# eyedealism/flexible-LLM-sharding

Measured on AMD Instinct MI355X. Metric: tokens/sec + peak GPU mem, Llama-2-70B layer_num_per_shard=1 at 1/2/4/8 MI355X, higher is better.
Workload: dtype fp16

## Files before the change

csrc/include/fls.h:

```cpp
#pragma once
#include <stdint.h>
#include <stddef.h>

#ifdef __cplusplus
extern "C" {
#endif

typedef void* fls_stream_t;

int   fls_rt_version(void);
void* fls_pinned_alloc(uint64_t bytes);
int   fls_pinned_free(void* p);
void* fls_host_device_ptr(void* p);
int   fls_pinned_register(void* p, uint64_t bytes);
int   fls_pinned_unregister(void* p);
int   fls_memcpy_async(void* dst, const void* src, uint64_t bytes, int kind, fls_stream_t s);
int64_t fls_pread_into(const char* path, uint64_t offset, uint64_t bytes, void* dst, int nthreads);
int64_t fls_pwrite_from(const char* path, uint64_t offset, uint64_t bytes, const void* src,
                        int nthreads, int truncate);
int   fls_gather_blocks(void* dst, const void* src, uint64_t block_bytes, const int64_t* src_block,
                        int64_t n_blocks, int nthreads);
void* fls_st_open(const char* path);
int   fls_st_count(void* h);
int   fls_st_info(void* h, int i, char* name, int name_cap, char* dtype, int dtype_cap,
// ... 50 lines not shown
int fls_moe_router_route(const void* h, int ldh, const void* wr, int ldw, int T, int H, int E, int k, int norm,
                         int round16, int* ids, float* w, fls_stream_t s);
int fls_moe_plan_scratch(int n, int E);
int fls_moe_plan(const int* ids, int n, int k, int E, int* offs, int* tiles, int* rows, int* dest, int* bhist,
                 fls_stream_t s);
int fls_moe_gemm(const void* A, const void* W, void* C, int M_bound, int N, int K, int lda, int ldw, int ldc, int epi,
                 const int* tiles, const int* offs, const int* rows, int n_groups, long long wstride, int a_rows,
                 fls_stream_t s);
int fls_moe_combine(const void* y, int ldy, const int* ids, const int* dest, const float* w, void* x, int ldx, int T,
                    int k, int H, const void* sh, int ldsh, fls_stream_t s);
int fls_gemm_set_order(int order);
int fls_gemm_set_mid_bn(int bn);
int fls_gemm_set_mid_waves(int waves);
int fls_gemm_set_mid_rows(int rows);
int fls_gemm_set_mid(int on);
int fls_attention_set_hpb(int hpb);
int fls_attention_set_split(int ns);
int fls_attention_set_persistent(int on);
int fls_attention(const void* qkv, void* out, const int* work, int n_items, int n_q_heads,
                  int n_kv_heads, int head_dim, int ld_qkv, int ld_out, float scale, const void* kv0,
                  int ld_kv0, const int* seg_lo, int q_block, const int* work2, const int* r2win,
                  void* ws, unsigned long long ws_bytes, int n_rows, fls_stream_t s);
int fls_attention_window(const void* qkv, void* out, const int* work, int n_items, int n_q_heads,
                         int n_kv_heads, int head_dim, int ld_qkv, int ld_out, float scale, const void* kv0,
                         int ld_kv0, const int* seg_lo, int q_block, const int* work2, const int* r2win,
                         void* ws, unsigned long long ws_bytes, int n_rows, const int* r0_lo,
                         const int* r0_item, fls_stream_t s);
int fls_headnorm_rope(void* x, int ldx, int rows, int n_q, int n_k, const void* qn, const void* kn, const int* pos,
                      const float* cos_t, const float* sin_t, int hd, float eps, fls_stream_t s);
int fls_rmsnorm(const void* x, const void* w, void* y, const int* row_idx, int rows, int H,
// ... 30 lines not shown
```

csrc/kernels/common.h:

```cpp
#pragma once
#include <hip/hip_runtime.h>
#include <stdint.h>

typedef _Float16 half_t;
typedef _Float16 half8 __attribute__((ext_vector_type(8)));
typedef _Float16 half4 __attribute__((ext_vector_type(4)));
typedef float floatx4 __attribute__((ext_vector_type(4)));
typedef short s16x4 __attribute__((vector_size(8)));

#define LDS_AS __attribute__((address_space(3)))
#define GLB_AS __attribute__((address_space(1)))

constexpr int WAVE = 64;

__device__ __forceinline__ floatx4 mfma16x16x32(half8 a, half8 b, floatx4 c) {
  return __builtin_amdgcn_mfma_f32_16x16x32_f16(a, b, c, 0, 0, 0);
}

__device__ __forceinline__ void mfma_acc_inplace_ordered(floatx4& c, const half8& a, const half8& b) {
  asm volatile("v_mfma_f32_16x16x32_f16 %0, %1, %2, %0" : "+a"(c) : "v"(a), "v"(b) : "memory");
}

__device__ __forceinline__ void glds16(const void* gsrc, void* lds_wave_base) {
  __builtin_amdgcn_global_load_lds((const GLB_AS void*)gsrc, (LDS_AS void*)lds_wave_base, 16, 0, 0);
// ... 6 lines not shown

__device__ __forceinline__ float warp_max(float v) {
#pragma unroll
  for (int o = 32; o > 0; o >>= 1) v = fmaxf(v, __shfl_xor(v, o, 64));
  return v;
}

__device__ __forceinline__ float warp_sum(float v) {
#pragma unroll
  for (int o = 32; o > 0; o >>= 1) v += __shfl_xor(v, o, 64);
  return v;
}

__device__ __forceinline__ float fast_exp2(float x) { return __builtin_amdgcn_exp2f(x); }

__device__ __forceinline__ float silu(float x) { return x / (1.0f + __expf(-x)); }

#define FLS_CHECK_LAUNCH()                                  \
  do {                                                      \
    hipError_t _e = hipGetLastError();                      \
    if (_e != hipSuccess) return (int)_e;                   \
  } while (0)
```

csrc/kernels/gemm.hip:

```cpp
#include "gemm_v10.h"

namespace {

template <int EPI>
__global__ __launch_bounds__(256) void gemm_nt_generic(const half_t* __restrict__ A, const half_t* __restrict__ W,
                                                     half_t* __restrict__ C, int M, int N, int K, int lda, int ldw,
                                                     int ldc, Epi ep) {
  const int lane = threadIdx.x & 63, wave = threadIdx.x >> 6;
  const int fr = lane & 15, grp = lane >> 4;
  const int m0 = blockIdx.x * 32;
  const bool rope128 = EPI == FLS_EPI_ROPE;
  const int gbase = blockIdx.y * 256 + (wave >> 1) * 128;
  int ncol[4];
#pragma unroll
  for (int t = 0; t < 4; ++t) ncol[t] = gbase + sub_col(rope128, wave & 1, t);
  floatx4 acc[2][4];
#pragma unroll
  for (int u = 0; u < 2; ++u)
#pragma unroll
    for (int t = 0; t < 4; ++t) acc[u][t] = floatx4{0.f, 0.f, 0.f, 0.f};
  for (int k0 = 0; k0 < K; k0 += 32) {
    half8 wf[4], xf[2];
    const int kb = k0 + grp * 8;
#pragma unroll
// ... 269 lines not shown
      const half4 b = *(const half4*)(ep.bias + col);
#pragma unroll
      for (int r = 0; r < 4; ++r) a[r] += (float)b[r];
    }
  };
  auto store4 = [&](const floatx4& a, int col) {
    half4 o;
#pragma unroll
    for (int r = 0; r < 4; ++r) o[r] = (half_t)a[r];
    *(half4*)(C + (size_t)m * ldc + col) = o;
  };
  if constexpr (EPI == FLS_EPI_SWIGLU) {
    const int I = N / 2;
    if (c >= I) return;
    const floatx4 g = sum4(c), u = sum4(I + c);
    floatx4 o;
#pragma unroll
    for (int r = 0; r < 4; ++r) o[r] = silu(g[r]) * u[r];
    store4(o, c);
  } else if constexpr (is_rope(EPI)) {
    const int hd = ep.head_dim, half_hd = hd >> 1, d = c % hd;
    if (c < ep.rope_cols && d >= half_hd) return;
    floatx4 a = sum4(c);
    bias4(a, c);
    if (c >= ep.rope_cols) {
      store4(a, c);
      return;
    }
    floatx4 b = sum4(c + half_hd);
    bias4(b, c + half_hd);
    const int p = ep.pos[m];
    const floatx4 cs = *(const floatx4*)(ep.cos_t + (size_t)p * half_hd + d);
    const floatx4 sn = *(const floatx4*)(ep.sin_t + (size_t)p * half_hd + d);
// ... 194 lines not shown
    return 0;
  }
  const int tiles = (int)tiles256;
  const int tiles_m = (M + BM - 1) / BM, tiles_n = N / BN;
  int order = g_order;
  if (order == 0) order = auto_order(tiles_m, tiles_n);
  Epi e = ep;
  e.order = order;
  launch_main<EPI>(tiles, A, W, C, M, N, K, lda, ldw, ldc, e, s);
  FLS_CHECK_LAUNCH();
  return 0;
}

}

extern "C" int fls_kernels_version(void) { return 41; }

extern "C" int fls_gemm_set_order(int order) {
  const int old = g_order;
  g_order = order;
  return old;
}

extern "C" int fls_gemm_set_skinny(int mode, int blocks) {
  const int old = g_skinny;
  g_skinny = mode < 0 ? 0 : mode > 2 ? 2 : mode;
  g_skinny_blocks = blocks > 0 ? blocks : 0;
  return old;
}

extern "C" int fls_gemm_set_skinny_bn(int bn) {
// ... 41 lines not shown
  const int old = g_mid_waves;
  g_mid_waves = waves == 4 || waves == 8 ? waves : 0;
  return old;
}

extern "C" int fls_gemm_set_mid_rows(int rows) {
  const int old = g_mid_rows;
  g_mid_rows = rows == 64 || rows == 128 ? rows : 0;
  return old;
}

extern "C" int fls_gemm_set_mid(int on) {
  const int old = g_mid;
  g_mid = on ? 1 : 0;
  return old;
}

extern "C" int fls_gemm_v11_try(const void* A, const void* W, void* C, const void* R, int M, int N, int K, int lda,
                                int ldw, int ldc, int ldr, int epi, const int* pos, const float* cos_t,
                                const float* sin_t, int rope_cols, int head_dim, const void* bias,
                                const float* rscale, float alpha, float* ss, int ss_ld, fls_stream_t s);

extern "C" int fls_gemm(const void* A, const void* W, void* C, const void* R, int M, int N, int K, int lda, int ldw,
                        int ldc, int ldr, int epi, const int* pos, const float* cos_t, const float* sin_t,
                        int rope_cols, int head_dim, const void* bias, const float* rscale, float alpha, float* ss,
                        int ss_ld, void* ws, uint64_t ws_bytes, fls_stream_t s) {
  if (M <= 0 || N <= 0 || K <= 0) return 0;
  const int row_exact = (epi & FLS_GEMM_ROW_EXACT) ? 1 : 0;
  epi &= 0xff;
  if (ss && (epi != FLS_EPI_RESID || N % 128 || ss_ld < N / 128)) return -7;
// ... 1 lines not shown
  if ((epi == FLS_EPI_SWIGLU || epi == FLS_EPI_ROPE) && (N % 32)) return -2;
  if (epi == FLS_EPI_ROPE && ((head_dim != 64 && head_dim != 128) || rope_cols % head_dim || N % head_dim))
    return -3;
  {
    const int rc = fls_gemm_v11_try(A, W, C, R, M, N, K, lda, ldw, ldc, ldr, epi, pos, cos_t, sin_t, rope_cols,
                                    head_dim, bias, rscale, alpha, ss, ss_ld, s);
    if (rc) return rc > 0 ? 0 : rc;
  }
  Epi ep{(const half_t*)R, ldr, pos, cos_t, sin_t, rope_cols, head_dim, (const half_t*)bias, N / 2, 0,
         nullptr, nullptr, nullptr, 0, 0};
  ep.rs = rscale;
  ep.alpha = alpha;
  ep.ss = ss;
  ep.ss_ld = ss_ld;
  ep.row_exact = row_exact;
  auto a = (const half_t*)A;
  auto w = (const half_t*)W;
  auto c = (half_t*)C;
  auto st = (hipStream_t)s;
  switch (epi) {
    case FLS_EPI_NONE: return launch<FLS_EPI_NONE>(a, w, c, M, N, K, lda, ldw, ldc, ep, st, ws, ws_bytes);
    case FLS_EPI_RESID: return launch<FLS_EPI_RESID>(a, w, c, M, N, K, lda, ldw, ldc, ep, st, ws, ws_bytes);
    case FLS_EPI_SWIGLU: return launch<FLS_EPI_SWIGLU>(a, w, c, M, N, K, lda, ldw, ldc, ep, st, ws, ws_bytes);
    case FLS_EPI_ROPE:
      return head_dim == 128 ? launch<FLS_EPI_ROPE>(a, w, c, M, N, K, lda, ldw, ldc, ep, st, ws, ws_bytes)
                             : launch<EPI_ROPE64>(a, w, c, M, N, K, lda, ldw, ldc, ep, st, ws, ws_bytes);
  }
  return -1;
}
```

csrc/kernels/gemm_skinny.h:

```cpp
namespace sk {
constexpr int KT = 64;
constexpr int LDS_MAX = 160 * 1024;
template <int RS, int BN>
struct Geo {
  static constexpr bool LATE = BN == 256;
  static constexpr int NSUB = BN / 64;
  static constexpr int XST = RS * 16 * KT * 2;
  static constexpr int WST = BN * KT * 2;
  static constexpr int STG = XST + WST;
  static constexpr int NX = 4 * STG <= LDS_MAX ? 4 : 3 * STG <= LDS_MAX ? 3 : 2;
  static constexpr int DIST = LATE ? NX - 1 : NX - 2;
  static constexpr int QX = RS / 2;
  static constexpr int QW = BN / 32;
  static constexpr int LDS = NX * STG;
  static_assert(DIST >= 1, "at least one K-tile in flight");
};
}

template <int RS, int EPI, int BN>
__global__ __launch_bounds__(256) void gemm_nt_skinny(const half_t* __restrict__ A, const half_t* __restrict__ W,
                                                      half_t* __restrict__ C, int M, int N, int K, int lda, int ldw,
                                                      int ldc, Epi ep) {
  using namespace sk;
  using G = Geo<RS, BN>;
// ... 89 lines not shown
  asm volatile("s_nop 7\n\ts_nop 7\n\ts_nop 7" ::: "memory");
#undef SK_FENCE_ACC

#pragma unroll
  for (int i = 0; i < RS; ++i) {
    const int m = i * 16 + fr;
    if (m >= M) continue;
    const float rsc = row_scale(ep, m);
    if constexpr (EPI == EPI_F32) {
      float* Cf = (float*)C + (size_t)blockIdx.y * ep.part_stride + (size_t)m * ldc;
#pragma unroll
      for (int j = 0; j < NS; ++j) *(floatx4*)(Cf + cbase + 16 * j + 4 * grp) = acc[i][j];
    } else if constexpr (EPI == FLS_EPI_SWIGLU) {
#pragma unroll
      for (int j = 0; j < NS / 2; ++j) {
        half4 o;
#pragma unroll
        for (int r = 0; r < 4; ++r) o[r] = (half_t)(silu(acc[i][j][r] * rsc) * (acc[i][j + NS / 2][r] * rsc));
        *(half4*)(C + (size_t)m * ldc + cbase + 16 * j + 4 * grp) = o;
      }
    } else {
#pragma unroll
      for (int j = 0; j < NS; ++j) {
        const int n = cbase + 16 * j + 4 * grp;
        floatx4 a = acc[i][j] * rsc;
        if (ep.bias) {
          const half4 b = *(const half4*)(ep.bias + n);
#pragma unroll
          for (int r = 0; r < 4; ++r) a[r] += (float)b[r];
        }
        if constexpr (EPI == FLS_EPI_RESID) {
          const half4 rr = *(const half4*)(ep.R + (size_t)m * ep.ldr + n);
#pragma unroll
// ... 113 lines not shown
```

csrc/kernels/gemm_v10.h:

```cpp
#pragma once
#include "common.h"
#include "fls.h"

#include <cstdlib>
#include <type_traits>

namespace {


constexpr int BM = 256, BN = 256, BK = 64;
constexpr int EPI_ROPE64 = 4;
constexpr int EPI_F32 = 6;
constexpr bool is_rope(int epi) { return epi == FLS_EPI_ROPE || epi == EPI_ROPE64; }
constexpr int BUF = 65536;
constexpr int WIMG = 32768;

struct Epi {
  const half_t* R;
  int ldr;
  const int* pos;
  const float* cos_t;
  const float* sin_t;
  int rope_cols;
  int head_dim;
// ... 1 lines not shown
  int gu_rows;
  int order;
  const int* g_tiles;
  const int* g_offs;
  const int* g_rows;
  long long g_wstride;
  int g_n;
  int ksplit;
  int kslice;
  long long part_stride;
  const float* rs = nullptr;
  float alpha = 1.f;
  float* ss = nullptr;
  int ss_ld = 0;
  int row_exact = 0;
};

__device__ __forceinline__ float row_sum_4groups(float v) {
  const auto a = __builtin_amdgcn_permlane32_swap(__float_as_uint(v), __float_as_uint(v), false, false);
  v = __uint_as_float(a[0]) + __uint_as_float(a[1]);
  const auto b = __builtin_amdgcn_permlane16_swap(__float_as_uint(v), __float_as_uint(v), false, false);
  return __uint_as_float(b[0]) + __uint_as_float(b[1]);
}

__device__ __forceinline__ float ss_accum_pair(float sq, const half4& oa, const half4& ob) {
#pragma unroll
  for (int r = 0; r < 4; ++r) {
    const float a = (float)oa[r], b = (float)ob[r];
    sq = __builtin_fmaf(a, a, sq);
    sq = __builtin_fmaf(b, b, sq);
// ... 2 lines not shown
}

__device__ __forceinline__ float row_scale(const Epi& ep, int m) { return ep.rs ? ep.rs[m] : 1.f; }

__device__ __forceinline__ int gu_phys_row(int l, int I) {
  return ((l >> 4) & 1) * I + (l >> 5) * 16 + (l & 15);
}

template <int EPI>
__device__ __forceinline__ void store_pair_off(half_t* __restrict__ C, int ldc, int m, int n_first, int off,
                                               const floatx4& acc_a, const floatx4& acc_b, const Epi& ep) {
  const int c0 = n_first + off;
  if constexpr (EPI == FLS_EPI_SWIGLU) {
    const int oc = n_first / 2 + off;
    const float s = row_scale(ep, m);
    half4 o;
#pragma unroll
    for (int r = 0; r < 4; ++r) o[r] = (half_t)(silu(acc_a[r] * s) * (acc_b[r] * s));
    *(half4*)(C + (size_t)m * ldc + oc) = o;
    return;
  } else {
    const float s = row_scale(ep, m);
    floatx4 a = acc_a * s, b = acc_b * s;
    if (ep.bias) {
      const half4 ba = *(const half4*)(ep.bias + c0);
      const half4 bb = *(const half4*)(ep.bias + c0 + 16);
#pragma unroll
      for (int r = 0; r < 4; ++r) { a[r] += (float)ba[r]; b[r] += (float)bb[r]; }
    }
    if constexpr (EPI == FLS_EPI_RESID) {
      const half4 ra = *(const half4*)(ep.R + (size_t)m * ep.ldr + c0);
      const half4 rb = *(const half4*)(ep.R + (size_t)m * ep.ldr + c0 + 16);
#pragma unroll
// ... 54 lines not shown
  const auto r1 = __builtin_amdgcn_permlane16_swap(v.y, v.w, false, false);
  a = __builtin_bit_cast(half4, uint2{r0[0], r1[0]});
  b = __builtin_bit_cast(half4, uint2{r0[1], r1[1]});
}

template <int HD, int U = 8, bool LO = false>
__device__ __forceinline__ void epilogue_rope(half_t* __restrict__ C, int ldc, int M, int mrow0, int ncol0, int grp,
                                              floatx4 (&acc)[U][8], const Epi& ep, int mlo = 0) {
  constexpr int HS = HD / 32;
  constexpr int HALF = HD / 2;
  const int off = 4 * grp;
  const int woff = wide_off(grp);
  int pos[U];
#pragma unroll
  for (int u = 0; u < U; ++u) pos[u] = ep.pos[min(mrow0 + u * 16, M - 1)];
  const float* const rsp = ep.rs;
  int f0[4];
  bool rot[4];
  half4 ba[4], bb[4];
#pragma unroll
  for (int q = 0; q < 4; ++q) {
    const int ta = HD == 128 ? q : (q & 1) + (q >> 1) * 4;
    const int ca = ncol0 + ta * 16;
    f0[q] = (ta * 16) % HD + off;
    rot[q] = ca < ep.rope_cols;
    if (ep.bias) {
      ba[q] = *(const half4*)(ep.bias + ca + off);
      bb[q] = *(const half4*)(ep.bias + ca + HALF + off);
    } else {
      ba[q] = half4{0, 0, 0, 0};
      bb[q] = half4{0, 0, 0, 0};
// ... 4 lines not shown
#pragma unroll
    for (int q = 0; q < 4; ++q) {
      if (rot[q]) {
        cs[sl][q] = *(const floatx4*)(ep.cos_t + (size_t)pos[u] * HALF + f0[q]);
        sn[sl][q] = *(const floatx4*)(ep.sin_t + (size_t)pos[u] * HALF + f0[q]);
      }
    }
  };
  load(0, 0);
#pragma unroll
  for (int u = 0; u < U; ++u) {
    const int sl = u & 1;
    if (u + 1 < U) load(u + 1, sl ^ 1);
    asm volatile("" ::: "memory");
    const int m = mrow0 + u * 16;
    const float s = rsp ? rsp[min(m, M - 1)] : 1.f;
    half4 oa[4], ob[4];
#pragma unroll
    for (int q = 0; q < 4; ++q) {
      const int ta = HD == 128 ? q : (q & 1) + (q >> 1) * 4;
#pragma unroll
      for (int r = 0; r < 4; ++r) {
        float x1 = __builtin_fmaf(acc[u][ta][r], s, (float)ba[q][r]);
        float x2 = __builtin_fmaf(acc[u][ta + HS][r], s, (float)bb[q][r]);
        if (rot[q]) {
          const float c = cs[sl][q][r], sv = sn[sl][q][r];
          const float y1 = __builtin_fmaf(x1, c, -(x2 * sv)), y2 = __builtin_fmaf(x2, c, x1 * sv);
          x1 = y1;
          x2 = y2;
        }
        oa[q][r] = (half_t)x1;
// ... 26 lines not shown
#pragma unroll
        for (int t = 0; t < 8; ++t) *(floatx4*)(Cf + (size_t)m * ldc + ncol0 + t * 16 + 4 * grp) = acc[u][t];
      }
    }
    return;
  } else if constexpr (EPI == FLS_EPI_ROPE) {
    epilogue_rope<128, U, LO>(C, ldc, M, mrow0, ncol0, grp, acc, ep, mlo);
    return;
  } else if constexpr (EPI == EPI_ROPE64) {
    epilogue_rope<64, U, LO>(C, ldc, M, mrow0, ncol0, grp, acc, ep, mlo);
    return;
  } else {
    const int off = 4 * grp;
    const int woff = wide_off(grp);
    if constexpr (EPI == FLS_EPI_SWIGLU) {
#pragma unroll
      for (int u = 0; u < U; ++u) {
        const int m = mrow0 + u * 16;
        const float s = ep.rs ? ep.rs[min(m, M - 1)] : 1.f;
        half4 o[4];
#pragma unroll
        for (int p = 0; p < 4; ++p)
#pragma unroll
          for (int r = 0; r < 4; ++r) o[p][r] = (half_t)(silu(acc[u][2 * p][r] * s) * (acc[u][2 * p + 1][r] * s));
#pragma unroll
        for (int p = 0; p < 4; p += 2) {
          const uint4 v = wide_pair(o[p], o[p + 1]);
          if (m < M && (!LO || m >= mlo)) *(uint4*)(C + (size_t)m * ldc + ncol0 / 2 + p * 16 + woff) = v;
        }
      }
      return;
    } else {
      half4 ba[4], bb[4];
#pragma unroll
      for (int p = 0; p < 4; ++p) {
        if (ep.bias) {
          ba[p] = *(const half4*)(ep.bias + ncol0 + p * 32 + off);
          bb[p] = *(const half4*)(ep.bias + ncol0 + p * 32 + off + 16);
        } else {
// ... 176 lines not shown
  _Pragma("unroll") for (int i_ = 0; i_ < 4; ++i_)                                                \
    V10_DMA_X(rA, k0, (hb) * 4 + i_, smem + (buf) * BUF + (prow[i_] + (hb) * 64) * 128);
#define V10_W(buf, hb, k0)                                                                         \
  _Pragma("unroll") for (int i_ = 0; i_ < 4; ++i_)                                                \
    V10_DMA_W(rW, hb, i_, k0, smem + (buf) * BUF + WIMG + (prow[i_] + (hb) * 64) * 128);

  const int wm = wave >> 1, wn = wave & 1;
  const int fr = lane & 15, grp = lane >> 4;
  const int sw = fr & 7;
  const int c0 = ((0 + grp) ^ sw) << 4;
  const int c1 = ((4 + grp) ^ sw) << 4;
  const int xrow = (wm * 128 + fr) * 128;
  const int wrow = WIMG + (wn * 128 + fr) * 128;

  floatx4 acc[8][8];
#pragma unroll
  for (int u = 0; u < 8; ++u)
#pragma unroll
    for (int t = 0; t < 8; ++t) acc[u][t] = floatx4{0.f, 0.f, 0.f, 0.f};
  half8 xf[8][2], wf[8][2];
#define V10_FENCE_ACC()                                                                            \
  _Pragma("unroll") for (int u_ = 0; u_ < 8; ++u_)                                                \
  _Pragma("unroll") for (int t_ = 0; t_ < 8; ++t_) asm volatile("" : "+a"(acc[u_][t_]));
  V10_FENCE_ACC();
  asm volatile("s_nop 7\n\ts_nop 7" ::: "memory");

#define V10_RX(buf, h)                                                                             \
  _Pragma("unroll") for (int u_ = (h) * 4; u_ < (h) * 4 + 4; ++u_) {                              \
    xf[u_][0] = *(const half8*)(smem + (buf) * BUF + xrow + u_ * 2048 + c0);                      \
    xf[u_][1] = *(const half8*)(smem + (buf) * BUF + xrow + u_ * 2048 + c1);                      \
  }
#define V10_RW(buf, h)                                                                             \
  _Pragma("unroll") for (int t_ = (h) * 4; t_ < (h) * 4 + 4; ++t_) {                              \
    wf[t_][0] = *(const half8*)(smem + (buf) * BUF + wrow + t_ * 2048 + c0);                      \
    wf[t_][1] = *(const half8*)(smem + (buf) * BUF + wrow + t_ * 2048 + c1);                      \
  }
#define V10_PHASE(xh, wh, RX, rbuf, rh, DX, dbuf, dhb, dk0, SYNC)                                  \
  {                                                                                               \
    _Pragma("unroll") for (int i_ = 0; i_ < 32; ++i_) {                                           \
      const int s_ = i_ >> 4, u_ = (xh) * 4 + ((i_ >> 2) & 3), t_ = (wh) * 4 + (i_ & 3);          \
// ... 13 lines not shown
        else                                                                                      \
          V10_DMA_W(rW##dk0, dhb, p_, dk0, smem + (dbuf) * BUF + WIMG + (prow[p_] + (dhb) * 64) * 128); \
      }                                                                                           \
    }                                                                                             \
    if (SYNC) {                                                                                   \
      __builtin_amdgcn_s_waitcnt(0xC07F);                                         \
      asm volatile("s_waitcnt vmcnt(16)" ::: "memory");                                           \
      __builtin_amdgcn_s_barrier();                                                               \
    }                                                                                             \
  }

  const int nk = K / BK;
  const int kc1 = min(1, nk - 1) * BK;
  V10_X(0, 0, 0); V10_W(0, 0, 0); V10_W(0, 1, 0); V10_X(0, 1, 0);
  V10_X(1, 0, kc1); V10_W(1, 1, kc1); V10_W(1, 0, kc1); V10_X(1, 1, kc1);
  asm volatile("s_waitcnt vmcnt(24)" ::: "memory");
  __builtin_amdgcn_s_barrier();
  V10_RX(0, 0); V10_RW(0, 0);
  __builtin_amdgcn_s_waitcnt(0xC07F);
  asm volatile("s_waitcnt vmcnt(16)" ::: "memory");
  __builtin_amdgcn_s_barrier();
  for (int kt = 0; kt < nk; kt += 2) {
    const int ka = min(kt + 2, nk - 1) * BK;
    const int kb = min(kt + 3, nk - 1) * BK;
    const __amdgpu_buffer_rsrc_t rXka = kt + 2 < nk ? rA : rZ, rWka = kt + 2 < nk ? rW : rZ;
    const __amdgpu_buffer_rsrc_t rXkb = kt + 3 < nk ? rA : rZ, rWkb = kt + 3 < nk ? rW : rZ;
    V10_PHASE(0, 0, 0, 0, 1, 1, 0, 0, ka, 0);
    V10_PHASE(0, 1, 1, 0, 1, 0, 0, 0, ka, 1);
    V10_PHASE(1, 1, 1, 1, 0, 0, 0, 1, ka, 0);
    V10_PHASE(1, 0, 0, 1, 1, 1, 0, 1, ka, 1);
// ... 33 lines not shown
```

csrc/kernels/gemm_v11.hip:

```cpp
#include "gemm_v10.h"


namespace {
namespace v11 {
constexpr int TM = 384, TN = 256, TK = 64;
constexpr int X01_0 = 0, X01_STG = 32768;
constexpr int X2_0 = 65536, X2_STG = 16384;
constexpr int W_0 = 98304, W_STG = 32768;
constexpr int LDS_BYTES = 163840;
}

__device__ __forceinline__ void mfma_acc_v_ordered(floatx4& c, const half8& a, const half8& b) {
  asm volatile("v_mfma_f32_16x16x32_f16 %0, %1, %2, %0" : "+v"(c) : "v"(a), "v"(b) : "memory");
}

template <int EPI>
__global__ __launch_bounds__(256, 1) void gemm_nt_v11(const half_t* __restrict__ A, const half_t* __restrict__ W,
                                                    half_t* __restrict__ C, int M, int N, int K, int lda, int ldw,
                                                    int ldc, Epi ep) {
  using namespace v11;
  extern __shared__ __attribute__((aligned(16))) char smem[];
  const int tid = threadIdx.x;
  const int lane = tid & 63;
  const int wave = __builtin_amdgcn_readfirstlane(tid >> 6);
// ... 45 lines not shown
      xso[j][i] + (unsigned)(k0) * 2u, 0, 0)
#define V11_DMA_W(rs, buf, i, k0)                                                                  \
  __builtin_amdgcn_raw_ptr_buffer_load_lds(rs, (LDS_AS void*)(smem + W_0 + (buf) * W_STG + (8 * wave + (i)) * 1024), \
                                           16, wl, wso[i] + (unsigned)(k0) * 2u, 0, 0)

  const int wm = wave >> 1, wn = wave & 1;
  const int fr = lane & 15, grp = lane >> 4;
  const int sw = fr & 7;
  const int cs0 = ((0 + grp) ^ sw) << 4;
  const int cs1 = ((4 + grp) ^ sw) << 4;
  const int xrow = X01_0 + (wm * 128 + fr) * 128;
  const int x2row = X2_0 + (wm * 64 + fr) * 128;
  const int wrow = W_0 + (wn * 128 + fr) * 128;

  floatx4 acc[8][8], accv[4][8];
#pragma unroll
  for (int u = 0; u < 8; ++u)
#pragma unroll
    for (int t = 0; t < 8; ++t) acc[u][t] = floatx4{0.f, 0.f, 0.f, 0.f};
#pragma unroll
  for (int u = 0; u < 4; ++u)
#pragma unroll
    for (int t = 0; t < 8; ++t) accv[u][t] = floatx4{0.f, 0.f, 0.f, 0.f};
  half8 xf[12], wf[8];
#define V11_FENCE_ACC()                                                                            \
  _Pragma("unroll") for (int u_ = 0; u_ < 8; ++u_)                                                \
  _Pragma("unroll") for (int t_ = 0; t_ < 8; ++t_) asm volatile("" : "+a"(acc[u_][t_]));          \
  _Pragma("unroll") for (int u_ = 0; u_ < 4; ++u_)                                                \
  _Pragma("unroll") for (int t_ = 0; t_ < 8; ++t_) asm volatile("" : "+v"(accv[u_][t_]));
  V11_FENCE_ACC();
  asm volatile("s_nop 7\n\ts_nop 7" ::: "memory");

  const char* const bx01_0 = smem + xrow + cs0;
  const char* const bx01_1 = smem + xrow + cs1;
  const char* const bx2_0 = smem + x2row + cs0;
  const char* const bx2_1 = smem + x2row + cs1;
  const char* const bw_0 = smem + wrow + cs0;
  const char* const bw_1 = smem + wrow + cs1;
#define V11_RX(f, buf, s)                                                                          \
  xf[f] = (f) < 8 ? *(const half8*)(((s) ? bx01_1 : bx01_0) + (buf) * X01_STG + (f) * 2048)        \
                  : *(const half8*)(((s) ? bx2_1 : bx2_0) + (buf) * X2_STG + ((f) - 8) * 2048)
#define V11_RW(t, buf, s) wf[t] = *(const half8*)(((s) ? bw_1 : bw_0) + (buf) * W_STG + (t) * 2048)
#define V11_MFMA(u, t)                                                                             \
  do {                                                                                            \
    if ((u) < 8) mfma_acc_inplace_ordered(acc[(u) & 7][t], wf[t], xf[u]);                         \
    else mfma_acc_v_ordered(accv[(u) & 3][t], wf[t], xf[u]);                                      \
// ... 48 lines not shown
#pragma unroll
    for (int i = 0; i < 4; ++i) V11_DMA_X(rA, 0, 0, i, 0);
#pragma unroll
    for (int i = 0; i < 4; ++i) V11_DMA_X(rA, 0, 1, i, 0);
#pragma unroll
    for (int i = 0; i < 8; ++i) V11_DMA_W(rW, 0, i, 0);
#pragma unroll
    for (int i = 0; i < 4; ++i) V11_DMA_X(rA, 0, 2, i, 0);
#pragma unroll
    for (int i = 0; i < 4; ++i) V11_DMA_X(rA, 1, 0, i, k1);
#pragma unroll
    for (int i = 0; i < 4; ++i) V11_DMA_X(rA, 1, 1, i, k1);
#pragma unroll
    for (int i = 0; i < 4; ++i) V11_DMA_W(rW, 1, i, k1);
  }
  asm volatile("s_waitcnt vmcnt(12)" ::: "memory");
  __builtin_amdgcn_s_barrier();
#pragma unroll
  for (int u = 0; u < 8; ++u) V11_RX(u, 0, 0);
#pragma unroll
  for (int t = 0; t < 8; ++t) V11_RW(t, 0, 0);

  for (int kt = 0; kt < nk; kt += 2) {
    const int k1 = min(kt + 1, nk - 1) * TK, k2 = min(kt + 2, nk - 1) * TK, k3 = min(kt + 3, nk - 1) * TK;
    const __amdgpu_buffer_rsrc_t rX1 = kt + 1 < nk ? rA : rZA;
    const __amdgpu_buffer_rsrc_t rX2 = kt + 2 < nk ? rA : rZA, rW2 = kt + 2 < nk ? rW : rZW;
    const __amdgpu_buffer_rsrc_t rX3 = kt + 3 < nk ? rA : rZA, rW3 = kt + 3 < nk ? rW : rZW;
    const __amdgpu_buffer_rsrc_t rW1 = kt + 1 < nk ? rW : rZW;
#define V11_TILE(B, rXn, rWn, kn, rXf, rWf, kf)                                                    \
  {                                                                                               \
// ... 9 lines not shown
    V11_PHASE_C(B, 1, dX0a, 2);                                                        \
    V11_PHASE_A(B, 1, (B) ^ 1, 0, dX0b, 2);                                            \
    V11_SYNC(6, 4);                                                                     \
    V11_PHASE_B(B, 1, (B) ^ 1, 0, dX1, 4);                                             \
    V11_PHASE_C((B) ^ 1, 0, dWlo, 4);                                                  \
    V11_SYNC(8, 12);                                                                    \
  }
    V11_TILE(0, rX1, rW1, k1, rX2, rW2, k2);
    V11_TILE(1, rX2, rW2, k2, rX3, rW3, k3);
#undef V11_TILE
  }
  asm volatile("s_waitcnt vmcnt(0)" ::: "memory");
  asm volatile("s_nop 7\n\ts_nop 7\n\ts_nop 7" ::: "memory");
  V11_FENCE_ACC();
#undef V11_FENCE_ACC
#undef V11_RX
#undef V11_RW
#undef V11_MFMA
#undef V11_DMA_AT
#undef V11_DMAS
#undef V11_SYNC
#undef V11_PHASE_A
#undef V11_PHASE_B
#undef V11_PHASE_C
#undef V11_DMA_X
#undef V11_DMA_W

  const int mrow = m0 + wm * 192 + fr, ncol = n0 + wn * 128;
  epilogue_quadrant<EPI, 4, true>(C, ldc, M, mrow + 128, ncol, grp, accv, ep, mlo);
  epilogue_quadrant<EPI, 8, true>(C, ldc, M, mrow, ncol, grp, acc, ep, mlo);
// ... 57 lines not shown
  if (!g_v11 || M < TM || N % TN || K % TK || (K / TK) % 2 || lda % 8 || ldw % 8) return 0;
  if (g_v11 == 1) {
    if ((size_t)((M + TM - 1) / TM) * (N / TN) < 256 || !v11_pays(M, N)) return 0;
  }
  if ((size_t)M * lda * 2 >= (1ull << 32)) return 0;
  if (epi == FLS_EPI_SWIGLU && (size_t)(N / 2 + TN) * ldw * 2 >= (1ull << 32)) return 0;
  if ((size_t)N * ldw * 2 >= (1ull << 32)) return 0;
  if (ldc % 8 || ((uintptr_t)C & 15)) return 0;
  if (epi == FLS_EPI_RESID && (ldr % 8 || ((uintptr_t)R & 15))) return 0;
  Epi ep{(const half_t*)R, ldr, pos, cos_t, sin_t, rope_cols, head_dim, (const half_t*)bias, N / 2, 0,
         nullptr, nullptr, nullptr, 0, 0};
  ep.rs = rscale;
  ep.alpha = alpha;
  ep.ss = ss;
  ep.ss_ld = ss_ld;
  auto a = (const half_t*)A;
  auto w = (const half_t*)W;
  auto c = (half_t*)C;
  auto st = (hipStream_t)s;
  int rc;
  switch (epi) {
    case FLS_EPI_NONE: rc = launch_v11<FLS_EPI_NONE>(a, w, c, M, N, K, lda, ldw, ldc, ep, st); break;
    case FLS_EPI_RESID: rc = launch_v11<FLS_EPI_RESID>(a, w, c, M, N, K, lda, ldw, ldc, ep, st); break;
    case FLS_EPI_SWIGLU: rc = launch_v11<FLS_EPI_SWIGLU>(a, w, c, M, N, K, lda, ldw, ldc, ep, st); break;
    case FLS_EPI_ROPE:
      rc = head_dim == 128 ? launch_v11<FLS_EPI_ROPE>(a, w, c, M, N, K, lda, ldw, ldc, ep, st)
                           : launch_v11<EPI_ROPE64>(a, w, c, M, N, K, lda, ldw, ldc, ep, st);
      break;
    default: return 0;
  }
// ... 3 lines not shown
```

csrc/kernels/moe.hip:

```cpp
#include "gemm_v10.h"

namespace {

constexpr int ROUTE_WAVES = 4;
constexpr int MAX_E = 256;
constexpr int MAX_K = 8;

__device__ __forceinline__ void wave_argmax(float& v, int& i) {
#pragma unroll
  for (int o = 32; o > 0; o >>= 1) {
    const float ov = __shfl_xor(v, o, 64);
    const int oi = __shfl_xor(i, o, 64);
    if (ov > v || (ov == v && oi < i)) {
      v = ov;
      i = oi;
    }
  }
}

__device__ __forceinline__ void route_token(const float (&l)[4], int lane, int E, int k, int norm, int round16,
                                            size_t t, int* __restrict__ ids, float* __restrict__ w) {
  float mx = -INFINITY;
#pragma unroll
  for (int q = 0; q < 4; ++q) mx = fmaxf(mx, l[q]);
// ... 249 lines not shown
}

template <int EPI>
int launch_grouped(const half_t* A, const half_t* W, half_t* C, int M_bound, int N, int K, int lda, int ldw,
                   int ldc, const int* tiles, const int* offs, const int* rows, int n_groups, long long wstride,
                   hipStream_t s) {
  static bool attr = false;
  if (!attr) {
    (void)hipFuncSetAttribute((const void*)gemm_nt_v10<EPI, true>, hipFuncAttributeMaxDynamicSharedMemorySize,
                              2 * BUF);
    attr = true;
  }
  const int tiles_m = (M_bound + BM - 1) / BM, tiles_n = N / BN;
  Epi ep{nullptr, 0, nullptr, nullptr, nullptr, 0, 0, nullptr, N / 2, auto_order(tiles_m, tiles_n),
         tiles, offs, rows, wstride, n_groups};
  hipLaunchKernelGGL((gemm_nt_v10<EPI, true>), dim3(tiles_m * tiles_n), dim3(256), 2 * BUF, s, A, W, C, M_bound, N,
                     K, lda, ldw, ldc, ep);
  FLS_CHECK_LAUNCH();
  return 0;
}

}

extern "C" int fls_moe_route(const void* logits, int ldl, int T, int E, int k, int norm, int round16, int* ids,
                             float* w, fls_stream_t s) {
  if (T <= 0) return 0;
  if (E < 1 || E > MAX_E || k < 1 || k > MAX_K || k > E) return -2;
  hipLaunchKernelGGL(moe_route_kernel, dim3((T + ROUTE_WAVES - 1) / ROUTE_WAVES), dim3(ROUTE_WAVES * 64), 0,
                     (hipStream_t)s, (const half_t*)logits, ldl, T, E, k, norm, round16, ids, w);
  FLS_CHECK_LAUNCH();
// ... 66 lines not shown
```

flexible_llm_sharding_amd/_native/__init__.py:

```python
from __future__ import annotations

import ctypes
import os
import threading

HERE = os.path.dirname(os.path.abspath(__file__))
_KERNELS = os.path.join(HERE, "libfls_kernels.so")
_RUNTIME = os.path.join(HERE, "libfls_runtime.so")
_COMM = os.path.join(HERE, "libfls_comm.so")

_lock = threading.Lock()
_libs = {}

c_void_p, c_int, c_int64, c_uint64, c_float, c_char_p = (
    ctypes.c_void_p, ctypes.c_int, ctypes.c_int64, ctypes.c_uint64, ctypes.c_float, ctypes.c_char_p)


def _bind(lib, name, restype, *argtypes):
    f = getattr(lib, name)
    f.restype = restype
    f.argtypes = list(argtypes)


def _load_runtime():
# ... 20 lines not shown
    _bind(lib, "fls_streamer_create", c_void_p, c_int, c_uint64, c_int, c_int, c_int)
    _bind(lib, "fls_streamer_pinned_bytes", c_uint64, c_void_p)
    _bind(lib, "fls_streamer_load", c_int64, c_void_p, c_char_p, c_void_p, c_int, c_void_p, c_void_p)
    _bind(lib, "fls_stream_read_host", c_int64, c_char_p, c_void_p, c_int, c_void_p, c_int)
    _bind(lib, "fls_streamer_stats", c_int, c_void_p, c_void_p, c_void_p, c_void_p, c_void_p, c_void_p)
    _bind(lib, "fls_streamer_destroy", None, c_void_p)
    _bind(lib, "fls_f32_to_f16", None, c_void_p, c_void_p, c_uint64)
    return lib


class Piece(ctypes.Structure):
    _fields_ = [("file_off", ctypes.c_uint64), ("nbytes", ctypes.c_uint64), ("dst_off", ctypes.c_uint64),
                ("kind", ctypes.c_int32), ("pad", ctypes.c_int32)]


KERNELS_ABI = 41


def _load_kernels(path: str = _KERNELS):
    lib = ctypes.CDLL(path)
    _bind(lib, "fls_kernels_version", c_int)
    if lib.fls_kernels_version() != KERNELS_ABI:
        raise RuntimeError(f"{path} is a stale build (ABI {lib.fls_kernels_version()} != {KERNELS_ABI}); "
                           "rebuild with python -m flexible_llm_sharding_amd._native.build")
    _bind(lib, "fls_gemm", c_int, c_void_p, c_void_p, c_void_p, c_void_p, c_int, c_int, c_int,
          c_int, c_int, c_int, c_int, c_int, c_void_p, c_void_p, c_void_p, c_int, c_int, c_void_p, c_void_p,
          c_float, c_void_p, c_int, c_void_p, c_uint64, c_void_p)
    _bind(lib, "fls_rstd_from_ss", c_int, c_void_p, c_int, c_int, c_int, c_int, c_float, c_void_p, c_void_p)
    _bind(lib, "fls_row_ss", c_int, c_void_p, c_int, c_int, c_int, c_void_p, c_int, c_void_p)
    _bind(lib, "fls_row_stat", c_int, c_void_p, c_int, c_int, c_int, c_float, c_void_p, c_void_p)
    _bind(lib, "fls_argmax_rows", c_int, c_void_p, c_int, c_int, c_int, c_void_p, c_void_p)
# ... 8 lines not shown
    _bind(lib, "fls_gemm_set_mid_waves", c_int, c_int)
    _bind(lib, "fls_gemm_set_mid_rows", c_int, c_int)
    _bind(lib, "fls_moe_route", c_int, c_void_p, c_int, c_int, c_int, c_int, c_int, c_int, c_void_p, c_void_p,
          c_void_p)
    _bind(lib, "fls_moe_router_route", c_int, c_void_p, c_int, c_void_p, c_int, c_int, c_int, c_int, c_int, c_int,
          c_int, c_void_p, c_void_p, c_void_p)
    _bind(lib, "fls_moe_plan_scratch", c_int, c_int, c_int)
    _bind(lib, "fls_moe_plan", c_int, c_void_p, c_int, c_int, c_int, c_void_p, c_void_p, c_void_p, c_void_p, c_void_p,
          c_void_p)
    _bind(lib, "fls_moe_gemm", c_int, c_void_p, c_void_p, c_void_p, c_int, c_int, c_int, c_int, c_int, c_int, c_int,
          c_void_p, c_void_p, c_void_p, c_int, ctypes.c_longlong, c_int, c_void_p)
    _bind(lib, "fls_moe_combine", c_int, c_void_p, c_int, c_void_p, c_void_p, c_void_p, c_void_p, c_int, c_int,
          c_int, c_int, c_void_p, c_int, c_void_p)
    _bind(lib, "fls_gemm_set_order", c_int, c_int)
    _bind(lib, "fls_gemm_set_v11", c_int, c_int)
    _bind(lib, "fls_gemm_set_v11_cost", c_int, c_int)
    _bind(lib, "fls_gemm_v11_pays", c_int, c_int, c_int)
    _bind(lib, "fls_gemm_set_skinny", c_int, c_int, c_int)
    _bind(lib, "fls_gemm_set_skinny_bn", c_int, c_int)
    _bind(lib, "fls_attention_set_hpb", c_int, c_int)
    _bind(lib, "fls_attention_set_split", c_int, c_int)
    _bind(lib, "fls_attention_set_persistent", c_int, c_int)
    _bind(lib, "fls_attention", c_int, c_void_p, c_void_p, c_void_p, c_int, c_int, c_int, c_int,
          c_int, c_int, c_float, c_void_p, c_int, c_void_p, c_int, c_void_p, c_void_p, c_void_p, c_uint64, c_int,
          c_void_p)
    _bind(lib, "fls_attention_window", c_int, c_void_p, c_void_p, c_void_p, c_int, c_int, c_int, c_int,
          c_int, c_int, c_float, c_void_p, c_int, c_void_p, c_int, c_void_p, c_void_p, c_void_p, c_uint64, c_int,
          c_void_p, c_void_p, c_void_p)
    _bind(lib, "fls_rmsnorm", c_int, c_void_p, c_void_p, c_void_p, c_void_p, c_int, c_int, c_int,
          c_int, c_float, c_void_p)
# ... 77 lines not shown
```

Baseline: 10030.

## Add fast packed SiLU in SwiGLU epilogues and overlap accumulator zeroing with DMA

Replaces the per-element SiLU in all SwiGLU GEMM epilogues with a packed two-wide exp2/rcp chain that uses Newton refinement. A wave-wide guard falls back to the reference expf formula when outputs are tiny or huge, so results stay bitwise equal to the reference. Also moves accumulator zeroing in the v10/v11 kernels after the first global-load issue, hides the zeroing latency behind DMA, and hoists the row-scale loads out of the epilogue loops. Adds a runtime toggle, an exhaustive on-device check kernel, and an ABI bump.

```diff
diff --git a/csrc/include/fls.h b/csrc/include/fls.h
--- a/csrc/include/fls.h
+++ b/csrc/include/fls.h
@@ -88,6 +88,8 @@
 int fls_gemm_set_mid_waves(int waves);
 int fls_gemm_set_mid_rows(int rows);
 int fls_gemm_set_mid(int on);
+int fls_gemm_set_silu(int mode);
+int fls_silu_check(uint32_t first_bits, uint64_t count, uint64_t* n_bad, uint32_t* first_bad, fls_stream_t s);
 int fls_attention_set_hpb(int hpb);
 int fls_attention_set_split(int ns);
 int fls_attention_set_persistent(int on);
diff --git a/csrc/kernels/common.h b/csrc/kernels/common.h
--- a/csrc/kernels/common.h
+++ b/csrc/kernels/common.h
@@ -44,7 +44,48 @@
 
 __device__ __forceinline__ float fast_exp2(float x) { return __builtin_amdgcn_exp2f(x); }
 
-__device__ __forceinline__ float silu(float x) { return x / (1.0f + __expf(-x)); }
+__device__ __forceinline__ float silu_ref(float x) { return x / (1.0f + __expf(-x)); }
+
+typedef float floatx2 __attribute__((ext_vector_type(2)));
+
+__device__ __forceinline__ floatx2 silu_chain2(floatx2 x) {
+#pragma clang fp contract(off)
+  const floatx2 t = x * floatx2{-0x1.715476p+0f, -0x1.715476p+0f};
+  const floatx2 e = floatx2{__builtin_amdgcn_exp2f(t.x), __builtin_amdgcn_exp2f(t.y)};
+  const floatx2 d = e + floatx2{1.0f, 1.0f};
+  const floatx2 r = floatx2{__builtin_amdgcn_rcpf(d.x), __builtin_amdgcn_rcpf(d.y)};
+  const floatx2 e0 = __builtin_elementwise_fma(-d, r, floatx2{1.0f, 1.0f});
+  const floatx2 r1 = __builtin_elementwise_fma(e0, r, r);
+  const floatx2 q = x * r1;
+  const floatx2 e1 = __builtin_elementwise_fma(-d, q, x);
+  const floatx2 q1 = __builtin_elementwise_fma(e1, r1, q);
+  const floatx2 e2 = __builtin_elementwise_fma(-d, q1, x);
+  return __builtin_elementwise_fma(e2, r1, q1);
+}
+
+constexpr float SILU_Y_MIN = 0x1p-100f;
+constexpr float SILU_Y_BIG = 0x1p+40f;
+
+template <int N>
+__device__ __forceinline__ void silu(const float (&x)[N], float (&y)[N], int fast) {
+  static_assert(N % 2 == 0, "silu: pairs");
+  if (fast) {
+    float mn = __builtin_inff();
+    floatx2 big = floatx2{0.f, 0.f};
+#pragma unroll
+    for (int i = 0; i < N; i += 2) {
+      const floatx2 v = silu_chain2(floatx2{x[i], x[i + 1]});
+      y[i] = v.x;
+      y[i + 1] = v.y;
+      mn = __builtin_fminf(__builtin_fminf(__builtin_fabsf(v.x), __builtin_fabsf(v.y)), mn);
+      big = __builtin_elementwise_fma(v, floatx2{SILU_Y_BIG, SILU_Y_BIG}, big);
+    }
+    const float g = __builtin_fmaf(big.x + big.y, 0.0f, mn);
+    if (!__any(!(g >= SILU_Y_MIN))) return;
+  }
+#pragma unroll
+  for (int i = 0; i < N; ++i) y[i] = silu_ref(x[i]);
+}
 
 #define FLS_CHECK_LAUNCH()                                  \
   do {                                                      \
diff --git a/csrc/kernels/gemm.hip b/csrc/kernels/gemm.hip
--- a/csrc/kernels/gemm.hip
+++ b/csrc/kernels/gemm.hip
@@ -1,6 +1,35 @@
 #include "gemm_v10.h"
 
+int g_fls_silu = 1;
+
 namespace {
+
+__global__ __launch_bounds__(256) void silu_check_kernel(unsigned first, unsigned long long count,
+                                                         unsigned long long* __restrict__ n_bad,
+                                                         unsigned* __restrict__ first_bad_off) {
+  const unsigned long long wave = __builtin_amdgcn_readfirstlane((int)((blockIdx.x * blockDim.x + threadIdx.x) >> 6));
+  const unsigned long long waves = (unsigned long long)gridDim.x * (blockDim.x >> 6);
+  unsigned bad = 0, bad_off = 0xffffffffu;
+  for (unsigned long long base = wave * 64; base < count; base += waves * 64) {
+    const int n = (int)(count - base < 64 ? count - base : 64);
+    for (int k = 0; k < n; ++k) {
+      const unsigned off = (unsigned)(base + k);
+      const float v = __uint_as_float(first + off);
+      const float x[2] = {v, v};
+      float y[2];
+      silu(x, y, 1);
+      const unsigned want = __float_as_uint(silu_ref(v));
+      if (__float_as_uint(y[0]) != want || __float_as_uint(y[1]) != want) {
+        ++bad;
+        bad_off = min(bad_off, off);
+      }
+    }
+  }
+  if ((threadIdx.x & 63) == 0 && bad) {
+    atomicAdd(n_bad, (unsigned long long)bad);
+    atomicMin(first_bad_off, bad_off);
+  }
+}
 
 template <int EPI>
 __global__ __launch_bounds__(256) void gemm_nt_generic(const half_t* __restrict__ A, const half_t* __restrict__ W,
@@ -307,9 +336,11 @@
     const int I = N / 2;
     if (c >= I) return;
     const floatx4 g = sum4(c), u = sum4(I + c);
+    float x[4] = {g[0], g[1], g[2], g[3]}, y[4];
+    silu(x, y, ep.silu_fast);
     floatx4 o;
 #pragma unroll
-    for (int r = 0; r < 4; ++r) o[r] = silu(g[r]) * u[r];
+    for (int r = 0; r < 4; ++r) o[r] = y[r] * u[r];
     store4(o, c);
   } else if constexpr (is_rope(EPI)) {
     const int hd = ep.head_dim, half_hd = hd >> 1, d = c % hd;
@@ -534,7 +565,7 @@
 
 }
 
-extern "C" int fls_kernels_version(void) { return 41; }
+extern "C" int fls_kernels_version(void) { return 42; }
 
 extern "C" int fls_gemm_set_order(int order) {
   const int old = g_order;
@@ -606,6 +637,40 @@
   const int old = g_mid;
   g_mid = on ? 1 : 0;
   return old;
+}
+
+extern "C" int fls_gemm_set_silu(int mode) {
+  const int old = g_fls_silu;
+  g_fls_silu = mode ? 1 : 0;
+  return old;
+}
+
+extern "C" int fls_silu_check(uint32_t first_bits, uint64_t count, uint64_t* n_bad, uint32_t* first_bad,
+                              fls_stream_t s) {
+  if (!n_bad || !first_bad || count > (1ull << 32)) return -2;
+  *n_bad = 0;
+  *first_bad = 0;
+  if (!count) return 0;
+  struct Res { unsigned long long n; unsigned off; unsigned pad; };
+  Res h{0, 0xffffffffu, 0}, *d = nullptr;
+  hipError_t e = hipMalloc((void**)&d, sizeof(Res));
+  if (e != hipSuccess) return (int)e;
+  const auto st = (hipStream_t)s;
+  e = hipMemcpyAsync(d, &h, sizeof(Res), hipMemcpyHostToDevice, st);
+  if (e == hipSuccess) {
+    const unsigned long long groups = (count + 63) / 64;
+    const unsigned blocks = (unsigned)(groups < 4 * 1024 ? (groups + 3) / 4 : 1024);
+    hipLaunchKernelGGL(silu_check_kernel, dim3(blocks), dim3(256), 0, st, (unsigned)first_bits,
+                       (unsigned long long)count, &d->n, &d->off);
+    e = hipGetLastError();
+  }
+  if (e == hipSuccess) e = hipMemcpyAsync(&h, d, sizeof(Res), hipMemcpyDeviceToHost, st);
+  if (e == hipSuccess) e = hipStreamSynchronize(st);
+  (void)hipFree(d);
+  if (e != hipSuccess) return (int)e;
+  *n_bad = h.n;
+  *first_bad = h.n ? first_bits + h.off : 0;
+  return 0;
 }
 
 extern "C" int fls_gemm_v11_try(const void* A, const void* W, void* C, const void* R, int M, int N, int K, int lda,
@@ -637,6 +702,7 @@
   ep.ss = ss;
   ep.ss_ld = ss_ld;
   ep.row_exact = row_exact;
+  ep.silu_fast = g_fls_silu;
   auto a = (const half_t*)A;
   auto w = (const half_t*)W;
   auto c = (half_t*)C;
diff --git a/csrc/kernels/gemm_skinny.h b/csrc/kernels/gemm_skinny.h
--- a/csrc/kernels/gemm_skinny.h
+++ b/csrc/kernels/gemm_skinny.h
@@ -127,9 +127,12 @@
     } else if constexpr (EPI == FLS_EPI_SWIGLU) {
 #pragma unroll
       for (int j = 0; j < NS / 2; ++j) {
+        const floatx4 g = acc[i][j] * rsc, up = acc[i][j + NS / 2] * rsc;
+        float x[4] = {g[0], g[1], g[2], g[3]}, y[4];
+        silu(x, y, ep.silu_fast);
         half4 o;
 #pragma unroll
-        for (int r = 0; r < 4; ++r) o[r] = (half_t)(silu(acc[i][j][r] * rsc) * (acc[i][j + NS / 2][r] * rsc));
+        for (int r = 0; r < 4; ++r) o[r] = (half_t)(y[r] * up[r]);
         *(half4*)(C + (size_t)m * ldc + cbase + 16 * j + 4 * grp) = o;
       }
     } else {
diff --git a/csrc/kernels/gemm_v10.h b/csrc/kernels/gemm_v10.h
--- a/csrc/kernels/gemm_v10.h
+++ b/csrc/kernels/gemm_v10.h
@@ -4,6 +4,8 @@
 
 #include <cstdlib>
 #include <type_traits>
+
+extern int g_fls_silu;
 
 namespace {
 
@@ -39,6 +41,7 @@
   float* ss = nullptr;
   int ss_ld = 0;
   int row_exact = 0;
+  int silu_fast = 1;
 };
 
 __device__ __forceinline__ float row_sum_4groups(float v) {
@@ -71,9 +74,12 @@
   if constexpr (EPI == FLS_EPI_SWIGLU) {
     const int oc = n_first / 2 + off;
     const float s = row_scale(ep, m);
+    const floatx4 g = acc_a * s, up = acc_b * s;
+    float x[4] = {g[0], g[1], g[2], g[3]}, y[4];
+    silu(x, y, ep.silu_fast);
     half4 o;
 #pragma unroll
-    for (int r = 0; r < 4; ++r) o[r] = (half_t)(silu(acc_a[r] * s) * (acc_b[r] * s));
+    for (int r = 0; r < 4; ++r) o[r] = (half_t)(y[r] * up[r]);
     *(half4*)(C + (size_t)m * ldc + oc) = o;
     return;
   } else {
@@ -158,7 +164,9 @@
   int pos[U];
 #pragma unroll
   for (int u = 0; u < U; ++u) pos[u] = ep.pos[min(mrow0 + u * 16, M - 1)];
-  const float* const rsp = ep.rs;
+  float rsc[U];
+#pragma unroll
+  for (int u = 0; u < U; ++u) rsc[u] = ep.rs ? ep.rs[min(mrow0 + u * 16, M - 1)] : 1.f;
   int f0[4];
   bool rot[4];
   half4 ba[4], bb[4];
@@ -193,7 +201,7 @@
     if (u + 1 < U) load(u + 1, sl ^ 1);
     asm volatile("" ::: "memory");
     const int m = mrow0 + u * 16;
-    const float s = rsp ? rsp[min(m, M - 1)] : 1.f;
+    const float s = rsc[u];
     half4 oa[4], ob[4];
 #pragma unroll
     for (int q = 0; q < 4; ++q) {
@@ -250,15 +258,28 @@
     const int off = 4 * grp;
     const int woff = wide_off(grp);
     if constexpr (EPI == FLS_EPI_SWIGLU) {
+      float rsc[U];
+#pragma unroll
+      for (int u = 0; u < U; ++u) rsc[u] = ep.rs ? ep.rs[min(mrow0 + u * 16, M - 1)] : 1.f;
 #pragma unroll
       for (int u = 0; u < U; ++u) {
         const int m = mrow0 + u * 16;
-        const float s = ep.rs ? ep.rs[min(m, M - 1)] : 1.f;
+        const float s = rsc[u];
+        float x[16], y[16];
+#pragma unroll
+        for (int p = 0; p < 4; ++p) {
+          const floatx4 g = acc[u][2 * p] * s;
+#pragma unroll
+          for (int r = 0; r < 4; ++r) x[4 * p + r] = g[r];
+        }
+        silu(x, y, ep.silu_fast);
         half4 o[4];
 #pragma unroll
-        for (int p = 0; p < 4; ++p)
-#pragma unroll
-          for (int r = 0; r < 4; ++r) o[p][r] = (half_t)(silu(acc[u][2 * p][r] * s) * (acc[u][2 * p + 1][r] * s));
+        for (int p = 0; p < 4; ++p) {
+          const floatx4 up = acc[u][2 * p + 1] * s;
+#pragma unroll
+          for (int r = 0; r < 4; ++r) o[p][r] = (half_t)(y[4 * p + r] * up[r]);
+        }
 #pragma unroll
         for (int p = 0; p < 4; p += 2) {
           const uint4 v = wide_pair(o[p], o[p + 1]);
@@ -465,16 +486,10 @@
   const int wrow = WIMG + (wn * 128 + fr) * 128;
 
   floatx4 acc[8][8];
-#pragma unroll
-  for (int u = 0; u < 8; ++u)
-#pragma unroll
-    for (int t = 0; t < 8; ++t) acc[u][t] = floatx4{0.f, 0.f, 0.f, 0.f};
   half8 xf[8][2], wf[8][2];
 #define V10_FENCE_ACC()                                                                            \
   _Pragma("unroll") for (int u_ = 0; u_ < 8; ++u_)                                                \
   _Pragma("unroll") for (int t_ = 0; t_ < 8; ++t_) asm volatile("" : "+a"(acc[u_][t_]));
-  V10_FENCE_ACC();
-  asm volatile("s_nop 7\n\ts_nop 7" ::: "memory");
 
 #define V10_RX(buf, h)                                                                             \
   _Pragma("unroll") for (int u_ = (h) * 4; u_ < (h) * 4 + 4; ++u_) {                              \
@@ -518,6 +533,13 @@
   const int kc1 = min(1, nk - 1) * BK;
   V10_X(0, 0, 0); V10_W(0, 0, 0); V10_W(0, 1, 0); V10_X(0, 1, 0);
   V10_X(1, 0, kc1); V10_W(1, 1, kc1); V10_W(1, 0, kc1); V10_X(1, 1, kc1);
+  __builtin_amdgcn_sched_barrier(0);
+#pragma unroll
+  for (int u = 0; u < 8; ++u)
+#pragma unroll
+    for (int t = 0; t < 8; ++t) acc[u][t] = floatx4{0.f, 0.f, 0.f, 0.f};
+  V10_FENCE_ACC();
+  asm volatile("s_nop 7\n\ts_nop 7" ::: "memory");
   asm volatile("s_waitcnt vmcnt(24)" ::: "memory");
   __builtin_amdgcn_s_barrier();
   V10_RX(0, 0); V10_RW(0, 0);
diff --git a/csrc/kernels/gemm_v11.hip b/csrc/kernels/gemm_v11.hip
--- a/csrc/kernels/gemm_v11.hip
+++ b/csrc/kernels/gemm_v11.hip
@@ -83,22 +83,27 @@
   const int wrow = W_0 + (wn * 128 + fr) * 128;
 
   floatx4 acc[8][8], accv[4][8];
-#pragma unroll
-  for (int u = 0; u < 8; ++u)
-#pragma unroll
-    for (int t = 0; t < 8; ++t) acc[u][t] = floatx4{0.f, 0.f, 0.f, 0.f};
-#pragma unroll
-  for (int u = 0; u < 4; ++u)
-#pragma unroll
-    for (int t = 0; t < 8; ++t) accv[u][t] = floatx4{0.f, 0.f, 0.f, 0.f};
   half8 xf[12], wf[8];
 #define V11_FENCE_ACC()                                                                            \
   _Pragma("unroll") for (int u_ = 0; u_ < 8; ++u_)                                                \
   _Pragma("unroll") for (int t_ = 0; t_ < 8; ++t_) asm volatile("" : "+a"(acc[u_][t_]));          \
   _Pragma("unroll") for (int u_ = 0; u_ < 4; ++u_)                                                \
   _Pragma("unroll") for (int t_ = 0; t_ < 8; ++t_) asm volatile("" : "+v"(accv[u_][t_]));
-  V11_FENCE_ACC();
-  asm volatile("s_nop 7\n\ts_nop 7" ::: "memory");
+#define V11_ZERO_ACC()                                                                             \
+  {                                                                                               \
+    _Pragma("unroll") for (int u_ = 0; u_ < 8; ++u_)                                              \
+    _Pragma("unroll") for (int t_ = 0; t_ < 8; ++t_) acc[u_][t_] = floatx4{0.f, 0.f, 0.f, 0.f};   \
+    _Pragma("unroll") for (int u_ = 0; u_ < 4; ++u_)                                              \
+    _Pragma("unroll") for (int t_ = 0; t_ < 8; ++t_) accv[u_][t_] = floatx4{0.f, 0.f, 0.f, 0.f};  \
+    V11_FENCE_ACC();                                                                              \
+    asm volatile("s_nop 7\n\ts_nop 7" ::: "memory");                                              \
+  }
+#ifndef FLS_V11_DMA_FIRST
+#define FLS_V11_DMA_FIRST 1
+#endif
+#if !FLS_V11_DMA_FIRST
+  V11_ZERO_ACC();
+#endif
 
   const char* const bx01_0 = smem + xrow + cs0;
   const char* const bx01_1 = smem + xrow + cs1;
@@ -177,6 +182,10 @@
 #pragma unroll
     for (int i = 0; i < 4; ++i) V11_DMA_W(rW, 1, i, k1);
   }
+#if FLS_V11_DMA_FIRST
+  __builtin_amdgcn_sched_barrier(0);
+  V11_ZERO_ACC();
+#endif
   asm volatile("s_waitcnt vmcnt(12)" ::: "memory");
   __builtin_amdgcn_s_barrier();
 #pragma unroll
@@ -216,6 +225,7 @@
   asm volatile("s_nop 7\n\ts_nop 7\n\ts_nop 7" ::: "memory");
   V11_FENCE_ACC();
 #undef V11_FENCE_ACC
+#undef V11_ZERO_ACC
 #undef V11_RX
 #undef V11_RW
 #undef V11_MFMA
@@ -303,6 +313,7 @@
   ep.alpha = alpha;
   ep.ss = ss;
   ep.ss_ld = ss_ld;
+  ep.silu_fast = g_fls_silu;
   auto a = (const half_t*)A;
   auto w = (const half_t*)W;
   auto c = (half_t*)C;
diff --git a/csrc/kernels/moe.hip b/csrc/kernels/moe.hip
--- a/csrc/kernels/moe.hip
+++ b/csrc/kernels/moe.hip
@@ -287,6 +287,7 @@
   const int tiles_m = (M_bound + BM - 1) / BM, tiles_n = N / BN;
   Epi ep{nullptr, 0, nullptr, nullptr, nullptr, 0, 0, nullptr, N / 2, auto_order(tiles_m, tiles_n),
          tiles, offs, rows, wstride, n_groups};
+  ep.silu_fast = g_fls_silu;
   hipLaunchKernelGGL((gemm_nt_v10<EPI, true>), dim3(tiles_m * tiles_n), dim3(256), 2 * BUF, s, A, W, C, M_bound, N,
                      K, lda, ldw, ldc, ep);
   FLS_CHECK_LAUNCH();
diff --git a/flexible_llm_sharding_amd/_native/__init__.py b/flexible_llm_sharding_amd/_native/__init__.py
--- a/flexible_llm_sharding_amd/_native/__init__.py
+++ b/flexible_llm_sharding_amd/_native/__init__.py
@@ -58,7 +58,7 @@
                 ("kind", ctypes.c_int32), ("pad", ctypes.c_int32)]
 
 
-KERNELS_ABI = 41
+KERNELS_ABI = 42
 
 
 def _load_kernels(path: str = _KERNELS):
@@ -97,6 +97,8 @@
           c_int, c_int, c_void_p, c_int, c_void_p)
     _bind(lib, "fls_gemm_set_order", c_int, c_int)
     _bind(lib, "fls_gemm_set_v11", c_int, c_int)
+    _bind(lib, "fls_gemm_set_silu", c_int, c_int)
+    _bind(lib, "fls_silu_check", c_int, ctypes.c_uint32, c_uint64, c_void_p, c_void_p, c_void_p)
     _bind(lib, "fls_gemm_set_v11_cost", c_int, c_int)
     _bind(lib, "fls_gemm_v11_pays", c_int, c_int, c_int)
     _bind(lib, "fls_gemm_set_skinny", c_int, c_int, c_int)
```

Result: no change. 10030 (median of 2 runs) (+0.0%).
